# floe/backscrub

Measured on AMD Instinct MI355X. Metric: composited frames/sec at 640×480 (batch), 1/2/4/8 MI355X + mask IoU vs CPU ref, higher is better.
Workload: dtype f32 (network) / u8 (image kernels); 1 GPU; BASELINE configs[1]: batch=256 640x480 frames, segm_lite_v681.tflite; moving scene: ring of 4 batches, a new one every step; 1 step = prep+network+decode+mask+blend, inputs resident in HBM; streams_per_gpu=256, library=bsx 0.1 (HIP gfx950, f32 NHWC)

## Files before the change

backscrub_amd/csrc/bsx_api.hip:

```cpp
#include "debug_switches.hpp"
#include <hip/hip_runtime.h>

#include <algorithm>
#include <cmath>
#include <cstdarg>
#include <cstdio>
#include <cstdlib>
#include <cstring>
#include <map>
#include <memory>
#include <string>
#include <thread>
#include <vector>

#include "../../include/bsx.h"
#include "gen_mid.hpp"
#include "kernels.hpp"
#include "roctx_ranges.hpp"
#include "plan.hpp"
#include "refusal.hpp"
#include "rtc.hpp"
#include "specialised.hpp"
#include "tflite_model.hpp"

// ... 1721 lines not shown
    if (!load_tflite(model_path, &g, &err) || !build_plan(g, &p, &err)) { snprintf(msg, cap, "%s", err.c_str()); return BSX_EMODEL; }
    if (p.program.empty()) { snprintf(msg, cap, "interpreted (no program)"); return BSX_OK; }
    const SpecialisedBuild b = build_specialised(p, kernel_variant(p), arch ? arch : "gfx950");
    const std::string& e = b.mid.fallback;
    if (b.mid.code.empty()) { snprintf(msg, cap, "%s", e.c_str()); return e.compare(0, 19, "interpreted (hipRTC") == 0 ? BSX_EMODEL : BSX_OK; }
    std::string seg_msg;
    if (p.seg.on) {
      if (!b.seg.code.empty()) {
        long worst = 0;
        for (const char* k : {"bsx_seg_head", "bsx_seg_k2", "bsx_seg_k3", "bsx_seg_tail"}) worst = std::max(worst, code_object_scratch_bytes(b.seg.code, k));
        char sm[256];
        snprintf(sm, sizeof sm, "; segment kernels %s (%zu bytes of source, %zu bytes of code object, %ld B of scratch)", b.seg.cached ? "cached" : "compiled", b.seg.source.size(),
                 b.seg.code.size(), worst);
        seg_msg = sm;
      } else {
        seg_msg = "; segment kernels: " + b.seg.fallback;
        if (b.seg.fallback.find("hipRTC:") != std::string::npos) { snprintf(msg, cap, "%s", seg_msg.c_str()); return BSX_EMODEL; }
      }
    }
    snprintf(msg, cap, "%s (%zu bytes of source, %zu bytes of code object, %ld B of scratch%s, cache %s)%s", b.mid.cached ? "cached" : "compiled", b.mid.source.size(),
             b.mid.code.size(), b.scratch, b.opaque_tid ? ", lane indices re-derived per op" : "", rtc_cache_dir().c_str(), seg_msg.c_str());
    return BSX_OK;
  } catch (...) { snprintf(msg, cap, "exception while reading the model"); return BSX_EMODEL; }
}

const char* bsx_plan_describe(bsx_ctx* c) { return c ? c->plan_text.c_str() : ""; }

static const char* debug_tensor_unstored(const bsx_ctx* c, int t) {
  const Plan& p = c->plan;
  if (t == p.input) return nullptr;
  if (t == p.output) return c->last_net_logits ? nullptr : "the last network stage decoded inside its final kernel and wrote no logits";
  if (c->use_program) {
    if (p.seg.on && std::find(p.seg_stored.begin(), p.seg_stored.end(), t) != p.seg_stored.end()) return nullptr;
    for (size_t i = 0; i < p.program.size() && i < p.program_out_tensor.size(); i++) {
      if (p.program_out_tensor[i] != t) continue;
      if (p.program[i].out.space == kLocLds) return "the frame program keeps it in LDS";
      if (p.program[i].out.space != kLocGlobal) return "the frame program writes it to a buffer of its own";
      if (program_op_elided(c, (int)i)) return "the specialised middle kernel computes it chunk by chunk inside the depthwise that reads it";
      return nullptr;
    }
    return p.seg.on ? "it lives inside a segment kernel or a fused micro-op (LDS / registers only)" : "it lives inside a fused micro-op (LDS / registers only)";
  }
  const int NS = (int)p.steps.size();
  const int n = c->last_net_n > 0 ? c->last_net_n : c->n_streams;
  const bool ir_on = c->d_weights16 && c->f16_terms > 0;
  for (int j = 0; j < NS; j++) {
    const Step& st = p.steps[j];
    if (st.out != t) continue;
    if (p.steps[0].fuse_head0 && j < 2) return "the fused head kernel (stem + depthwise + 1x1) keeps it in LDS";
    if (st.fuse_dw >= 0 && ir_on) return "the fused expand + depthwise kernel keeps it in LDS";
    if (st.chain_first >= 0 && chain3_on(p, j, n, c->d_weights16, c->f16_terms)) return "the chained 1x1 kernel keeps it in registers";
    if (st.chain_mid >= 0 && j < st.chain_mid && chain3_on(p, st.chain_mid, n, c->d_weights16, c->f16_terms)) return "the chained 1x1 kernel keeps it in registers";
    return nullptr;
  }
  return "no step of this plan writes it";
}

static long debug_tensor_at(bsx_ctx* c, int t, int stream_idx, float* h_out, long cap) {
  if (!c) return BSX_EINVAL;
  if (t < 0 || t >= (int)c->plan.tensor_off.size() || t >= (int)c->plan.tensor_elems.size() || stream_idx < 0 || stream_idx >= c->n_streams || (h_out && cap < 0)) { c->last_error = "bsx_debug_tensor: tensor or stream index out of range"; return BSX_EINVAL; }
  if (c->plan.tensor_off[t] < 0) { c->last_error = "bsx_debug_tensor: tensor " + std::to_string(t) + " has no place in the arena (a constant, or fused away by the planner)"; return BSX_EINVAL; }
  if (const char* why = debug_tensor_unstored(c, t)) { c->last_error = "bsx_debug_tensor: tensor " + std::to_string(t) + " is never written to the arena on this path: " + why; return BSX_EINVAL; }
  DeviceGuard guard(c->device);
  const long n = c->plan.tensor_elems[t];
  if (!h_out) return n;
  const float* p = (t == c->plan.input || t == c->plan.output || !c->use_program) ? c->tensor_ptr(t) + (size_t)stream_idx * (size_t)n
// ... 20 lines not shown
```

backscrub_amd/csrc/gen_seg.cpp:

```cpp
#include "gen_seg.hpp"

#include <cstdarg>
#include <cstdio>

namespace bsx {
namespace {

const char kSegSource[] =
#include "seg_rtc_src.inc"
    ;

}

std::string seg_constants_text(const SegPlan& sp, const char* pre) {
  std::string out;
  auto P = [&](const char* fmt, ...) {
    char buf[1024];
    va_list ap;
    va_start(ap, fmt);
    vsnprintf(buf, sizeof buf, fmt, ap);
    va_end(ap);
    out += buf;
  };
  auto conv = [&](const char* n, const SegConvW& c) { P("  t.%s.w_off = %lldll; t.%s.b_off = %lldll; t.%s.Cin = %d; t.%s.Cout = %d; t.%s.cout_pad = %d; t.%s.act = %d;\n", n, c.w_off, n, c.b_off, n, c.Cin, n, c.Cout, n, c.cout_pad, n, c.act); };
  auto dw = [&](const char* n, const SegDwW& c) { P("  t.%s.w_off = %lldll; t.%s.b_off = %lldll; t.%s.C = %d; t.%s.act = %d;\n", n, c.w_off, n, c.b_off, n, c.C, n, c.act); };
  auto gate = [&](const char* n, const SegGate& g_) {
    P("  t.%s.n_parts = %d; t.%s.sum_parts = %d; t.%s.n_fc = %d; t.%s.timing_skip = %d;\n", n, g_.n_parts, n, g_.sum_parts, n, g_.n_fc, n, g_.timing_skip);
    for (int i = 0; i < 2; i++) {
      P("  t.%s.part[%d].off = %lldll; t.%s.part[%d].n = %d; t.%s.part[%d].C = %d; t.%s.part[%d].hw = (float)%.9g;\n", n, i, g_.part[i].off, n, i, g_.part[i].n, n, i, g_.part[i].C, n, i, (double)g_.part[i].hw);
      P("  t.%s.fc[%d].w_off = %lldll; t.%s.fc[%d].b_off = %lldll; t.%s.fc[%d].Cin = %d; t.%s.fc[%d].Cout = %d; t.%s.fc[%d].act = %d;\n", n, i, g_.fc[i].w_off, n, i, g_.fc[i].b_off, n, i, g_.fc[i].Cin, n, i,
              g_.fc[i].Cout, n, i, g_.fc[i].act);
    }
  };
  auto end = [&](int dbg_skip) { if (dbg_skip) P("  t.dbg_skip = %d;\n", dbg_skip); P("  return t; }();\n"); };
  const SegHead& H = sp.head; const SegK2& K2 = sp.k2; const SegK3& K3 = sp.k3; const SegTail& T = sp.tail;
  P("// segment descriptors of the loaded graph as constants (gen_seg.cpp: seg_constants_text)\nconstexpr SegHead %sHEAD = [] { SegHead t{};\n", pre);
  P("  t.H0 = %d; t.W0 = %d; t.H1 = %d; t.W1 = %d; t.H2 = %d; t.W2 = %d; t.stem_pt = %d; t.stem_pl = %d; t.dw_pt = %d; t.dw_pl = %d;\n", H.H0, H.W0, H.H1, H.W1, H.H2, H.W2, H.stem_pt, H.stem_pl, H.dw_pt, H.dw_pl);
  conv("stem", H.stem); conv("pw", H.pw); dw("dw", H.dw);
  P("  t.a_off = %lldll; t.b0_off = %lldll; t.part_a_off = %lldll; t.part_b0_off = %lldll; t.TR = %d; t.TC = %d; t.tiles_y = %d; t.tiles_x = %d; t.lds_floats = %d; t.rw = %d; t.m_ct = %uu;\n",
          H.a_off, H.b0_off, H.part_a_off, H.part_b0_off, H.TR, H.TC, H.tiles_y, H.tiles_x, H.lds_floats, H.rw, H.m_ct);
  end(H.dbg_skip);
  P("constexpr SegK2 %sK2 = [] { SegK2 t{};\n  t.H2 = %d; t.W2 = %d; t.H3 = %d; t.W3 = %d; t.dw_pt = %d; t.dw_pl = %d;\n", pre, K2.H2, K2.W2, K2.H3, K2.W3, K2.dw_pt, K2.dw_pl);
  gate("gate", K2.gate); conv("pw_a", K2.pw_a); conv("pw_b", K2.pw_b); dw("dw", K2.dw);
  P("  t.b0_off = %lldll; t.B_off = %lldll; t.c0_off = %lldll; t.part_B_off = %lldll; t.TR = %d; t.TC = %d; t.tiles_y = %d; t.tiles_x = %d; t.lds_floats = %d; t.rw = %d; t.m_ct = %uu;\n",
          K2.b0_off, K2.B_off, K2.c0_off, K2.part_B_off, K2.TR, K2.TC, K2.tiles_y, K2.tiles_x, K2.lds_floats, K2.rw, K2.m_ct);
  end(K2.dbg_skip);
  P("constexpr SegK3 %sK3 = [] { SegK3 t{};\n  t.H2 = %d; t.W2 = %d; t.HL = %d; t.WL = %d; t.half_pixel = %d; t.align_corners = %d;\n", pre, K3.H2, K3.W2, K3.HL, K3.WL, K3.half_pixel, K3.align_corners);
  conv("pw1", K3.pw1); conv("pw2", K3.pw2); dw("dw", K3.dw);
  P("  t.skip_off = %lldll; t.lo2_off = %lldll; t.g_off = %lldll; t.lo_off = %lldll; t.part_lo_off = %lldll; t.TR = %d; t.TC = %d; t.tiles_y = %d; t.tiles_x = %d; t.lds_floats = %d; t.lo_floats = %d; t.hs = (float)%.9g; t.ws = (float)%.9g;\n",
          K3.skip_off, K3.lo2_off, K3.g_off, K3.lo_off, K3.part_lo_off, K3.TR, K3.TC, K3.tiles_y, K3.tiles_x, K3.lds_floats, K3.lo_floats, (double)K3.hs, (double)K3.ws);
  end(K3.dbg_skip);
  P("constexpr SegTail %sTAIL = [] { SegTail t{};\n  t.H1 = %d; t.W1 = %d; t.HL = %d; t.WL = %d; t.H0 = %d; t.W0 = %d; t.half_pixel = %d; t.align_corners = %d;\n", pre, T.H1, T.W1, T.HL, T.WL, T.H0, T.W0, T.half_pixel, T.align_corners);
  gate("gate", T.gate); conv("pw", T.pw); dw("dw", T.dw);
  P("  t.tc_w_off = %lldll; t.tc_b_off = %lldll; t.Co = %d; t.act3 = %d; t.model_type = %d; t.skip_off = %lldll; t.lo_off = %lldll; t.pre_gate_off = %lldll; t.TR = %d; t.TC = %d; t.tiles_y = %d; t.tiles_x = %d; "
             "t.lds_floats = %d; t.lo_floats = %d; t.hs = (float)%.9g; t.ws = (float)%.9g;\n",
          T.tc_w_off, T.tc_b_off, T.Co, T.act3, T.model_type, T.skip_off, T.lo_off, T.pre_gate_off, T.TR, T.TC, T.tiles_y, T.tiles_x, T.lds_floats, T.lo_floats, (double)T.hs, (double)T.ws);
  end(T.dbg_skip);
  return out;
}

std::string generate_seg_source(const Plan& plan, bool h16, bool u8in, std::string* why) {
  auto fail = [&](const char* m) { if (why) *why = m; return std::string(); };
  if (!plan.seg.on) return fail("no segment kernels in this plan");
  const SegPlan& sp = plan.seg;
  const bool sig = sp.tail.act3 == kActSigmoid;
  if (!((sp.tail.Co == 2 && !sig) || sp.tail.Co == 1)) return fail("transpose-convolution output channels");
  std::string src = kSegSource;
  const std::string mark = "BSXS_SEG_CONSTANTS";
  const size_t at = src.find(mark);
  if (at == std::string::npos) return fail("embedded source has no constants marker");
  src.replace(at, mark.size(), seg_constants_text(sp, "kSeg"));
  char head[512];
  snprintf(head, sizeof head, "#define BSXS_SEG_RTC 1\n#define BSXS_SEG_HS %d\n#define BSXS_SEG_H16 %d\n#define BSXS_SEG_U8 %d\n#define BSXS_SEG_SIG %d\n#define BSXS_SEG_CO %d\n",
           sp.head.stem.act == kActHswish ? 1 : 0, h16 ? 1 : 0, u8in ? 1 : 0, sig ? 1 : 0, sp.tail.Co);
  return std::string(head) + src;
}

}
// ... 1 lines not shown
```

backscrub_amd/csrc/kernels_seg.hip:

```cpp
#ifndef __HIPCC_RTC__
#include <hip/hip_runtime.h>
#endif
#ifndef BSX_SEG_RTC
#include "debug_switches.hpp"

#include <algorithm>
#include <cstdlib>
#include <type_traits>

#include "kernels.hpp"
#include "mfma_tile.hpp"
#include "segments.hpp"
#endif

#if defined(BSX_SEG_RTC)
#define BSX_SEG_D(T, NAME) constexpr T d = kSeg##NAME; (void)d_rt
#elif defined(BSX_SEG_PROBE)
#define BSX_SEG_D(T, NAME) constexpr T d = kProbe##NAME; (void)d_rt
#else
#define BSX_SEG_D(T, NAME) const T& d = d_rt
#endif

namespace bsx {
#ifdef BSX_SEG_RTC
// ... 47 lines not shown
  c.hi = act == kActRelu6 ? 6.f : __builtin_huge_valf();
  return c;
}
__device__ __forceinline__ float4 clamp4(float4 v, Clamp c) {
  return make_float4(__builtin_amdgcn_fmed3f(v.x, c.lo, c.hi), __builtin_amdgcn_fmed3f(v.y, c.lo, c.hi), __builtin_amdgcn_fmed3f(v.z, c.lo, c.hi),
                     __builtin_amdgcn_fmed3f(v.w, c.lo, c.hi));
}
__device__ __forceinline__ float hswish1(float v) { return v * __builtin_amdgcn_fmed3f(v + 3.f, 0.f, 6.f) * 0.16666667163372040f; }
__device__ __forceinline__ float4 hswish4(float4 v) { return make_float4(hswish1(v.x), hswish1(v.y), hswish1(v.z), hswish1(v.w)); }
__device__ __forceinline__ float sigmoid1(float v) { return __builtin_amdgcn_rcpf(1.f + __builtin_amdgcn_exp2f(v * -1.44269504088896341f)); }
__device__ __forceinline__ float sg_act(float v, int act) {
  if (act == kActNone) return v;
  if (act == kActSigmoid) return sigmoid1(v);
  if (act == kActHswish) return hswish1(v);
  if (act == kActRelu) return fmaxf(v, 0.f);
  return __builtin_amdgcn_fmed3f(v, 0.f, 6.f);
}

__device__ __forceinline__ float4 acc_quad(const f4acc acc) { return make_float4(acc[0], acc[1], acc[2], acc[3]); }
__device__ __forceinline__ f4acc mma16(const float4 a, const float (&wr)[4]) {
  f4acc acc = {0.f, 0.f, 0.f, 0.f};
  acc = __builtin_amdgcn_mfma_f32_16x16x4f32(wr[0], a.x, acc, 0, 0, 0);
  acc = __builtin_amdgcn_mfma_f32_16x16x4f32(wr[1], a.y, acc, 0, 0, 0);
  acc = __builtin_amdgcn_mfma_f32_16x16x4f32(wr[2], a.z, acc, 0, 0, 0);
  acc = __builtin_amdgcn_mfma_f32_16x16x4f32(wr[3], a.w, acc, 0, 0, 0);
  return acc;
}
__device__ __forceinline__ void load_wtile(float (&wr)[4], const float* __restrict__ w, const SegConvW& c, int n0, int li, int g) {
#pragma unroll
  for (int r = 0; r < 4; r++) wr[r] = (w + c.w_off)[(unsigned)((4 * g + r) * c.cout_pad + n0 + li)];
}

constexpr int kGateStageFloats = kSegGateStageFloats;
__device__ __forceinline__ void seg_gate(const SegGate& gt, const float* __restrict__ fa, const float* __restrict__ w, float* scr, float* stage) {
  float* s_gate = scr + kScrGate;
  if (gt.timing_skip) { if (threadIdx.x < 16) s_gate[threadIdx.x] = 0.5f; __syncthreads(); return; }
  float* s_mean = scr + kScrGate + 16;
  float* s_hid = scr + kScrGate + 48;
  const int tid = threadIdx.x;
  const SegFc &f1 = gt.fc[0], &f2 = gt.fc[1];
  const int w1n = f1.Cin * f1.Cout, w2n = gt.n_fc == 2 ? f2.Cin * f2.Cout : 0;
  float* ps = stage;
  float* w1 = ps + 512;
  float* b1 = w1 + w1n;
  float* w2 = b1 + f1.Cout;
  float* b2 = w2 + w2n;
  {
    const int c = tid & 15, slice = tid >> 4;
    for (int k = 0; k < gt.n_parts; k++) {
      const float* src = fa + gt.part[k].off;
      float s = 0.f;
#pragma unroll 4
      for (int i = slice; i < gt.part[k].n; i += 16) s += src[(unsigned)(i * 16 + c)];
      ps[k * 256 + slice * 16 + c] = s;
    }
  }
  {
    const float* g1 = w + f1.w_off;
    const float* g2 = w + f2.w_off;
    for (int i = tid; i < w1n; i += kSegThreads) w1[i] = g1[(unsigned)i];
    for (int i = tid; i < w2n; i += kSegThreads) w2[i] = g2[(unsigned)i];
    if (tid < f1.Cout) b1[tid] = (w + f1.b_off)[(unsigned)tid];
    if (gt.n_fc == 2 && tid < f2.Cout) b2[tid] = (w + f2.b_off)[(unsigned)tid];
  }
  __syncthreads();
  const int Cm = gt.sum_parts ? 16 : 16 * gt.n_parts;
  if (tid < Cm) {
    float m = 0.f;
    for (int k = 0; k < gt.n_parts; k++) {
      if (!gt.sum_parts && (tid >> 4) != k) continue;
      float s = 0.f;
#pragma unroll
      for (int sl = 0; sl < 16; sl++) s += ps[k * 256 + sl * 16 + (tid & 15)];
      m += s / gt.part[k].hw;
    }
    s_mean[tid] = m;
  }
  __syncthreads();
  auto fc = [&](const SegFc& f, const float* x, const float* wl, const float* bl, float* y) {
    const int out = tid >> 3, ks = tid & 7, kper = f.Cin >> 3;
    float acc = 0.f;
    if (out < f.Cout)
      for (int j = 0; j < kper; j++) acc = fmaf(x[ks * kper + j], wl[out * f.Cin + ks * kper + j], acc);
    acc += dpp_quad(acc, 1);
    acc += dpp_quad(acc, 2);
    acc += __builtin_bit_cast(float, __builtin_amdgcn_update_dpp(0, __builtin_bit_cast(int, acc), 0x141, 0xf, 0xf, true));
    if (out < f.Cout && ks == 0) y[out] = sg_act(acc + bl[out], f.act);
  };
  fc(f1, s_mean, w1, b1, gt.n_fc == 1 ? s_gate : s_hid);
  __syncthreads();
  if (gt.n_fc == 2) {
    fc(f2, s_hid, w2, b2, s_gate);
    __syncthreads();
  }
}

template <int SHR>
// ... 197 lines not shown
    for (int s7 = 0; s7 < 7; s7++) {
      acc0 = __builtin_amdgcn_mfma_f32_16x16x4f32(ws[s7], av0[s7], acc0, 0, 0, 0);
      acc1 = __builtin_amdgcn_mfma_f32_16x16x4f32(ws[s7], av1[s7], acc1, 0, 0, 0);
    }
    stem_pw_epilogue(acc0, r0t);
    if (two) stem_pw_epilogue(acc1, r1t);
  }
  const int quad = lane & 3, px = lane >> 2;
  f4v wd[9];
#pragma unroll
  for (int k = 0; k < 9; k++) wd[k] = ldv(w + d.dw.w_off + k * 16 + 4 * quad);
  const f4v bias_d = ldv(w + d.dw.b_off + 4 * quad);
  const int cox[3] = {(2 * px) * 16 + 4 * quad, (2 * px + 1) * 16 + 4 * quad, (2 * px + 2) * 16 + 4 * quad};
  __syncthreads();

  float4 sumB = f4zero();
  for (int py = wave; py < d.TR && !(d.dbg_skip & 4); py += 4) {
    if (r0 + py >= d.H2) break;
    if (px < d.TC && c0 + px < d.W2) {
      const float4 v = as_stored<H16>(clamp4(tof4(dw3x3(x_f, AC * 16, 2 * py, cox, wd) + bias_d), cl_dw));
      stg4<H16>(b0_out, (unsigned)(((r0 + py) * d.W2 + c0 + px) * 16 + 4 * quad), v);
      sumB = f4add(sumB, v);
    }
  }
  float* s_red = in_t;
  wave_reduce16<0>(sumA, s_red, wave, lane);
  wave_reduce16<1>(sumB, s_red + 256, wave, lane);
  __syncthreads();
  store_partials(s_red, fa + d.part_a_off + (long)t_ * 16);
  store_partials(s_red + 256, fa + d.part_b0_off + (long)t_ * 16);
}

#ifdef BSX_SEG_RTC
extern "C" __global__ __launch_bounds__(kSegThreads) __attribute__((amdgpu_waves_per_eu(6, 6))) void bsx_seg_k2(
#else
template <bool H16>
__global__ __launch_bounds__(kSegThreads) __attribute__((amdgpu_waves_per_eu(6, 6))) void seg_k2_k(
#endif
    const SegK2 d_rt, float* __restrict__ arena, long per_frame, const float* __restrict__ w, int n_frames) {
  BSX_SEG_D(SegK2, K2);
  unsigned f_, t_;
  xcd_frame_tile((unsigned)(d.tiles_y * d.tiles_x), (unsigned)n_frames, &f_, &t_);
  const int f = (int)f_, ty = (int)t_ / d.tiles_x, tx = (int)t_ - ty * d.tiles_x;
  const int r0 = ty * d.TR, c0 = tx * d.TC;
  const int BR = 2 * d.TR + 1, BC = 2 * d.TC + 1, br0 = 2 * r0 - d.dw_pt, bc0 = 2 * c0 - d.dw_pl, RW = d.rw, ctiles = RW >> 4;
  float* fa = arena + (size_t)f * (size_t)per_frame;
  float* B_t = seg_smem + kScrFloats;
  float* x_t = B_t + BR * RW * 16;
  const float* b0_in = fa + d.b0_off;
  float* B_out = fa + d.B_off;
  float* c0_out = fa + d.c0_off;
  const int tid = threadIdx.x, lane = tid & 63, wave = wave_uniform(tid >> 6), li = lane & 15, g = lane >> 4, cq4 = 4 * g;
  const int ntile = BR * ctiles, xe = li;
  const int la = col_a(li, g), lb = col_b(li, g, RW >> 1);
  constexpr int kB0 = 6;
  float4 b0v[kB0];
#pragma unroll
  for (int j = 0; j < kB0; j++) {
    const int t = wave + 4 * j;
    b0v[j] = f4zero();
    if (t < ntile) {
      const RowTile rt = row_tile(t, ctiles, d.m_ct);
      const int gy = br0 + rt.row, gx = bc0 + 16 * rt.ct + li;
      if (gy >= 0 && gy < d.H2 && gx >= 0 && gx < d.W2) b0v[j] = ldg4<H16>(b0_in, (unsigned)((gy * d.W2 + gx) * 16 + 4 * g));
    }
  }
  seg_gate(d.gate, fa, w, seg_smem, B_t);
  const float4 sv = ld4(seg_smem + kScrGate + 4 * g);
  float wr[4];
  load_wtile(wr, w, d.pw_a, 0, li, g);
  const float4 bias_a = ld4(w + d.pw_a.b_off + cq4);
  const Clamp cl_a = clamp_of(d.pw_a.act), cl_b = clamp_of(d.pw_b.act), cl_dw = clamp_of(d.dw.act);

  float4 sumB = f4zero();
#pragma unroll
  for (int j = 0; j < kB0; j++) {
    const int t = wave + 4 * j;
    if (t >= ntile) break;
    const RowTile rt = row_tile(t, ctiles, d.m_ct);
    float4 a = b0v[j];
    a = make_float4(__fmul_rn(a.x, sv.x), __fmul_rn(a.y, sv.y), __fmul_rn(a.z, sv.z), __fmul_rn(a.w, sv.w));
    const f4acc acc = mma16(a, wr);
    float4 v = acc_quad(acc);
    const int x2 = 16 * rt.ct + xe, hy = br0 + rt.row, hx = bc0 + x2;
    if (x2 < BC) {
      v = as_stored<H16>(clamp4(f4add(v, bias_a), cl_a));
      st4(B_t + (rt.row * RW + 16 * rt.ct) * 16 + la, v);
      const bool row_owned = hy >= max(2 * r0, 0) && hy < min(2 * r0 + 2 * d.TR, d.H2);
      if (row_owned && hx >= 2 * c0 && hx < min(2 * c0 + 2 * d.TC, d.W2)) {
        stg4<H16>(B_out, (unsigned)((hy * d.W2 + hx) * 16 + cq4), v);
        sumB = f4add(sumB, v);
      }
    }
  }
  float* s_red = seg_smem + kScrRed;
  wave_reduce16<0>(sumB, s_red, wave, lane);
  __syncthreads();
  store_partials(s_red, fa + d.part_B_off + (long)t_ * 16);

  const int C = d.dw.C, ngrp = (C + 15) >> 4, quad = lane & 3, px = lane >> 2;
  const int cox[3] = {col_b(2 * px, quad, RW >> 1), col_b(2 * px + 1, quad, RW >> 1), col_b(2 * px + 2, quad, RW >> 1)};
  for (int grp = 0; grp < ngrp && !(d.dbg_skip & 2); grp++) {
    load_wtile(wr, w, d.pw_b, 16 * grp, li, g);
    const float4 bias_b = ld4(w + d.pw_b.b_off + 16 * grp + cq4);
    for (int t = wave; t < ntile; t += 4) {
      const RowTile rt = row_tile(t, ctiles, d.m_ct);
      const f4acc acc = mma16(ld4(B_t + (rt.row * RW + 16 * rt.ct) * 16 + la), wr);
      float4 v = acc_quad(acc);
      const int x2 = 16 * rt.ct + xe, hy = br0 + rt.row, hx = bc0 + x2;
      if (x2 < BC) {
        const bool inside = hy >= 0 && hy < d.H2 && hx >= 0 && hx < d.W2;
        v = inside ? clamp4(f4add(v, bias_b), cl_b) : f4zero();
        st4(x_t + (rt.row * RW + 8 * rt.ct) * 16 + lb, v);
      }
    }
    const int ch = 16 * grp + 4 * quad;
    f4v wd[9];
    f4v bias_d = {0.f, 0.f, 0.f, 0.f};
    if (ch < C) {
#pragma unroll
      for (int k = 0; k < 9; k++) wd[k] = ldv(w + d.dw.w_off + (unsigned)(k * C + ch));
      bias_d = ldv(w + d.dw.b_off + ch);
    }
    __syncthreads();
    if (ch < C && px < d.TC && c0 + px < d.W3)
      for (int py = wave; py < d.TR && r0 + py < d.H3; py += 4) {
        const float4 v = clamp4(tof4(dw3x3(x_t, RW * 16, 2 * py, cox, wd) + bias_d), cl_dw);
        stg4<H16>(c0_out, (unsigned)(((r0 + py) * d.W3 + c0 + px) * C + ch), v);
      }
    __syncthreads();
  }
}

constexpr int kGatedRows = 5;
constexpr int kLoStride = kSegLoStride;
struct GatedPre { float4 s[kGatedRows]; int ly0, lx0, LC; };
template <bool H16>
__device__ __forceinline__ GatedPre gated_prefetch(const float* __restrict__ skip, const float* __restrict__ lo, int H, int W, int HL, int WL, bool half_pixel,
                                                   float hs, float wsc, int r0, int c0, int ZH, int ZC, float* l_t) {
  const int tid = threadIdx.x, lane = tid & 63, wave = wave_uniform(tid >> 6), li = lane & 15, g = lane >> 4;
  GatedPre pre;
  const int ix = c0 - 1 + li;
  const bool col_in = li < ZC && ix >= 0 && ix < W;
#pragma unroll
  for (int j = 0; j < kGatedRows; j++) {
    const int zy = wave + 4 * j, iy = r0 - 1 + zy;
    pre.s[j] = f4zero();
    if (zy < ZH && iy >= 0 && iy < H && col_in) pre.s[j] = ldg4<H16>(skip, (unsigned)((iy * W + ix) * 16 + 4 * g));
  }
  int ly0, ly1, lx0, lx1, t0, t1;
  float fr;
  up_axis(max(r0 - 1, 0), hs, half_pixel, HL, &ly0, &t1, &fr);
  up_axis(min(r0 - 2 + ZH, H - 1), hs, half_pixel, HL, &t0, &ly1, &fr);
  up_axis(max(c0 - 1, 0), wsc, half_pixel, WL, &lx0, &t1, &fr);
  up_axis(min(c0 - 2 + ZC, W - 1), wsc, half_pixel, WL, &t0, &lx1, &fr);
  const int LR = ly1 - ly0 + 1, LC = lx1 - lx0 + 1;
  pre.ly0 = ly0; pre.lx0 = lx0; pre.LC = LC;
  float4 v[3];
#pragma unroll
  for (int j = 0; j < 3; j++) {
    const int ly = wave + 4 * j;
    v[j] = f4zero();
// ... 265 lines not shown
```

backscrub_amd/csrc/plan.cpp:

```cpp
#include "debug_switches.hpp"
#include "plan.hpp"
#include "gen_seg.hpp"
#include "gen_mid.hpp"

#include <algorithm>
#include <cmath>
#include <cstdio>
#include <cstdlib>
#include <cstring>
#include <map>

namespace bsx {
namespace {

void conv_geometry(int in, int k, int s, int d, bool same, int* out, int* pad) {
  int eff = (k - 1) * d + 1;
  *out = same ? (in + s - 1) / s : (in + s - eff) / s;
  int total = (*out - 1) * s + eff - in;
  *pad = total > 0 ? total / 2 : 0;
}

uint16_t f32_to_f16_rn(float f) {
  uint32_t x; memcpy(&x, &f, 4);
  const uint32_t sign = (x >> 16) & 0x8000u;
// ... 564 lines not shown
  if (uses_of(B) != 3 || uses_of(up2) != 2 || uses_of(kp1.out) != 2 || uses_of(kd.out) != 1 || uses_of(kf2.out) != 1 || uses_of(lo) != 1 || uses_of(lo2) != 1) return seg_fail(21);
  if (!resize_weights_uniform(kr.H, kr.OH, kr.align_corners, kr.half_pixel) || !resize_weights_uniform(kr.W, kr.OW, kr.align_corners, kr.half_pixel)) return seg_fail(22);
  if (uses_of(c0) != 1) return seg_fail(23);
  auto clampish = [](int a) { return a == kActNone || a == kActRelu || a == kActRelu6; };
  if (!(clampish(stem.act) || stem.act == kActHswish) || !(ttc.act == kActNone || ttc.act == kActSigmoid) || (ttc.act == kActSigmoid && ttc.Cout != 1)) return seg_fail(34);
  for (const Step* q : {&hpw, &hdw, &pwa, &pwb, &kdw, &kp1, &kd, &kp2, &tpw, &tdw}) if (!clampish(q->act)) return seg_fail(35);

  size_t top = plan->arena_floats_per_stream;
  auto reserve = [&](size_t floats) { size_t at = top; top += (floats + 63) / 64 * 64; return (long long)at; };
  auto synth = [&](const char* name, int n, int C) {
    TensorInfo t; t.dims[0] = 1; t.dims[1] = n; t.dims[2] = 1; t.dims[3] = C; t.shape = {1, n, 1, C}; t.name = name;
    g.tensors.push_back(t);
    plan->tensor_off.push_back(-1);
    return (int)g.tensors.size() - 1;
  };
  SegPlan sp;
  int tgt[8] = {4, 14, 4, 7, 16, 14, 18, 14};
  if (const char* e = BSX_DBG_ENV("BSX_SEG_TILES")) sscanf(e, "%d,%d,%d,%d,%d,%d,%d,%d", &tgt[0], &tgt[1], &tgt[2], &tgt[3], &tgt[4], &tgt[5], &tgt[6], &tgt[7]);
  auto split = [&](int extent, int target, int* tile, int* n) { *n = tiles_for(extent, std::max(1, target)); *tile = (extent + *n - 1) / *n; };

  SegHead& h = sp.head;
  h.H0 = stem.H; h.W0 = stem.W; h.H1 = stem.OH; h.W1 = stem.OW; h.H2 = hdw.OH; h.W2 = hdw.OW;
  h.stem_pt = stem.pad_t; h.stem_pl = stem.pad_l; h.dw_pt = hdw.pad_t; h.dw_pl = hdw.pad_l;
  h.stem = conv_w(stem); h.pw = conv_w(hpw); h.dw = dw_w(hdw);
  split(h.H2, tgt[0], &h.TR, &h.tiles_y); split(h.W2, tgt[1], &h.TC, &h.tiles_x);
  h.lds_floats = seg_head_lds_floats(h);
  h.rw = seg_row_width(2 * h.TC + 1); h.m_ct = (65536u + (unsigned)(h.rw / 16) - 1) / (unsigned)(h.rw / 16);
  if (h.TR > 4 || h.TC > 15 || (4 * h.TC + 3) * 3 > 192) return seg_fail(30);
  SegK2& k2 = sp.k2;
  k2.H2 = hdw.OH; k2.W2 = hdw.OW; k2.H3 = kdw.OH; k2.W3 = kdw.OW; k2.dw_pt = kdw.pad_t; k2.dw_pl = kdw.pad_l;
  k2.pw_a = conv_w(pwa); k2.pw_b = conv_w(pwb); k2.dw = dw_w(kdw);
  split(k2.H3, tgt[2], &k2.TR, &k2.tiles_y); split(k2.W3, tgt[3], &k2.TC, &k2.tiles_x);
  k2.lds_floats = seg_k2_lds_floats(k2);
  k2.rw = seg_row_width(2 * k2.TC + 1); k2.m_ct = (65536u + (unsigned)(k2.rw / 16) - 1) / (unsigned)(k2.rw / 16);
  if (k2.TC > 15 || ((2 * k2.TR + 1) * (k2.rw / 16) + 3) / 4 > 6) return seg_fail(31);
  SegK3& k3 = sp.k3;
  k3.H2 = kp1.OH; k3.W2 = kp1.OW; k3.HL = kr.H; k3.WL = kr.W; k3.half_pixel = kr.half_pixel; k3.align_corners = kr.align_corners;
  k3.pw1 = conv_w(kp1); k3.pw2 = conv_w(kp2); k3.dw = dw_w(kd);
  split(k3.H2, tgt[4], &k3.TR, &k3.tiles_y); split(k3.W2, tgt[5], &k3.TC, &k3.tiles_x);
  k3.hs = seg_up_scale(k3.HL, k3.H2, k3.align_corners != 0); k3.ws = seg_up_scale(k3.WL, k3.W2, k3.align_corners != 0);
  if (!BSX_DBG_ENV("BSX_SEG_LO_WORST")) k3.lo_floats = seg_lo_window_floats(k3.H2, k3.W2, k3.HL, k3.WL, k3.half_pixel != 0, k3.align_corners != 0, k3.TR, k3.TC, k3.tiles_y, k3.tiles_x);
  k3.lds_floats = seg_k3_lds_floats(k3);
  if (k3.TC > 14 || k3.TR > 18) return seg_fail(32);
  SegTail& tl = sp.tail;
  tl.H1 = tpw.OH; tl.W1 = tpw.OW; tl.HL = tr.H; tl.WL = tr.W; tl.H0 = ttc.OH; tl.W0 = ttc.OW; tl.half_pixel = tr.half_pixel; tl.align_corners = tr.align_corners;
  tl.pw = conv_w(tpw); tl.dw = dw_w(tdw); tl.tc_w_off = (long long)ttc.w_off; tl.tc_b_off = (long long)ttc.b_off; tl.Co = ttc.Cout; tl.act3 = ttc.act;
  split(tl.H1, tgt[6], &tl.TR, &tl.tiles_y); split(tl.W1, tgt[7], &tl.TC, &tl.tiles_x);
  tl.hs = seg_up_scale(tl.HL, tl.H1, tl.align_corners != 0); tl.ws = seg_up_scale(tl.WL, tl.W1, tl.align_corners != 0);
  if (!BSX_DBG_ENV("BSX_SEG_LO_WORST")) tl.lo_floats = seg_lo_window_floats(tl.H1, tl.W1, tl.HL, tl.WL, tl.half_pixel != 0, tl.align_corners != 0, tl.TR, tl.TC, tl.tiles_y, tl.tiles_x);
  tl.lds_floats = seg_tail_lds_floats(tl);
  if (tl.TC > 14 || tl.TR > 18) return seg_fail(33);
  const int lds_cap = 160 * 256;
  if (h.lds_floats > lds_cap || k2.lds_floats > lds_cap || k3.lds_floats > lds_cap || tl.lds_floats > lds_cap) return seg_fail(24);
  if (ttc.OH != 2 * tpw.OH || ttc.OW != 2 * tpw.OW || h.H2 != k3.H2 || h.W2 != k3.W2) return seg_fail(25);
  if (h.tiles_y * h.tiles_x > 1024 || k2.tiles_y * k2.tiles_x > 1024 || k3.tiles_y * k3.tiles_x > 1024) return seg_fail(26);

  const int pA = synth("partials(A)", h.tiles_y * h.tiles_x, 16), pb0 = synth("partials(b0)", h.tiles_y * h.tiles_x, 16);
  const int pB = synth("partials(B)", k2.tiles_y * k2.tiles_x, 16), plo = synth("partials(lo)", k3.tiles_y * k3.tiles_x, 16);
  const int pgt = BSX_DBG_ENV("BSX_SEG_NO_GATE_KERNEL") ? -1 : synth("gate(tail)", 1, 16);
  if (pgt >= 0) plan->tensor_off[pgt] = reserve(16);
  for (int t : {A, b0, B, c0, lo2, lo, kf2.out, pA, pb0, pB, plo}) plan->tensor_off[t] = reserve(g.tensors[t].elems());
  for (int t : {hpw.out, g1.out, f1a.out, f1b.out, pwb.out, up2, kg.out, kf1.out, kp1.out, kd.out, up, tg.out, tf1.out, tf2.out, tpw.out, tdw.out})
    if (t != g.output) plan->tensor_off[t] = -1;
  plan->arena_floats_per_stream = top;
  plan->seg_stored = {A, b0, B, c0, lo};

  h.a_off = plan->tensor_off[A]; h.b0_off = plan->tensor_off[b0]; h.part_a_off = plan->tensor_off[pA]; h.part_b0_off = plan->tensor_off[pb0];
  k2.b0_off = plan->tensor_off[b0]; k2.B_off = plan->tensor_off[B]; k2.c0_off = plan->tensor_off[c0]; k2.part_B_off = plan->tensor_off[pB];
  k2.gate.n_parts = 1; k2.gate.n_fc = 2; k2.gate.sum_parts = 0;
  k2.gate.part[0].off = plan->tensor_off[pb0]; k2.gate.part[0].n = h.tiles_y * h.tiles_x; k2.gate.part[0].C = 16; k2.gate.part[0].hw = (float)(h.H2 * h.W2);
  k2.gate.fc[0] = fc_w(f1a); k2.gate.fc[1] = fc_w(f1b);
  k3.skip_off = plan->tensor_off[B]; k3.lo2_off = plan->tensor_off[lo2]; k3.g_off = plan->tensor_off[kf2.out]; k3.lo_off = plan->tensor_off[lo];
  k3.part_lo_off = plan->tensor_off[plo];
  tl.skip_off = plan->tensor_off[A]; tl.lo_off = plan->tensor_off[lo];
  tl.gate.n_parts = 2; tl.gate.n_fc = 2; tl.gate.sum_parts = tg.gap_sum ? 1 : 0;
  tl.gate.part[0].off = plan->tensor_off[pA]; tl.gate.part[0].n = h.tiles_y * h.tiles_x; tl.gate.part[0].C = 16; tl.gate.part[0].hw = (float)(h.H1 * h.W1);
  tl.gate.part[1].off = plan->tensor_off[plo]; tl.gate.part[1].n = k3.tiles_y * k3.tiles_x; tl.gate.part[1].C = 16; tl.gate.part[1].hw = (float)(k3.H2 * k3.W2);
  tl.gate.fc[0] = fc_w(tf1); tl.gate.fc[1] = fc_w(tf2);
  if (BSX_DBG_ENV("BSX_SEG_GATE_SKIP")) k2.gate.timing_skip = tl.gate.timing_skip = 1;
  if (const char* e = BSX_DBG_ENV("BSX_SEG_SKIP")) sscanf(e, "%d,%d,%d,%d", &h.dbg_skip, &k2.dbg_skip, &k3.dbg_skip, &tl.dbg_skip);
  tl.pre_gate_off = pgt >= 0 ? plan->tensor_off[pgt] : -1;
  if (tl.gate.fc[0].Cin != (tl.gate.sum_parts ? 16 : 32) || k2.gate.fc[0].Cin != 16) return seg_fail(27);

  std::vector<Step> mid(S.begin() + 9, S.begin() + (NS - 14));
  Step gate = kg;
  gate.concat_in = {B, lo2};
  gate.in0 = B;
  gate.label += "*";
  mid.push_back(gate); mid.push_back(kf1); mid.push_back(kf2);
  std::map<int, int> part_n, part_hw;
  part_n[B] = k2.tiles_y * k2.tiles_x; part_hw[B] = k2.H2 * k2.W2;
  const long B_real = plan->tensor_off[B];
  plan->tensor_off[B] = plan->tensor_off[pB];
  build_frame_program(g, plan, mid, {c0, B, lo2, kf2.out}, part_n, part_hw);
  plan->tensor_off[B] = B_real;
  if (plan->program.empty()) return seg_fail(28);
  sp.on = true;
  plan->seg = sp;
#ifdef BSX_DEBUG_SWITCHES
  if (const char* path = BSX_DBG_ENV("BSX_SEG_DUMP")) {
    if (FILE* f = fopen(path, "w")) { fputs(seg_constants_text(sp, "kProbe").c_str(), f); fclose(f); }
  }
#endif
  char line[256];
  plan->seg_text.clear();
  auto add = [&](const char* name, int TR, int TC, int ty, int tx, int lds, std::initializer_list<int> stores) {
    snprintf(line, sizeof line, "segment %-5s tile %dx%d, %dx%d tiles per frame, LDS %.1f KiB, stores", name, TR, TC, ty, tx, lds / 256.0);
    plan->seg_text += line;
    for (int t : stores) plan->seg_text += " t" + std::to_string(t);
    plan->seg_text += stores.size() ? "\n" : " the network output\n";
  };
  add("head", h.TR, h.TC, h.tiles_y, h.tiles_x, h.lds_floats, {A, b0}); add("k2", k2.TR, k2.TC, k2.tiles_y, k2.tiles_x, k2.lds_floats, {B, c0});
  add("k3", k3.TR, k3.TC, k3.tiles_y, k3.tiles_x, k3.lds_floats, {lo}); add("tail", tl.TR, tl.TC, tl.tiles_y, tl.tiles_x, tl.lds_floats, {});
  return true;
}


MidGeometry mid_geometry_default() {
  static const MidGeometry geo = [] {
    MidGeometry m{kFrameThreads, kLdsTotalFloats};
    if (const char* e = BSX_DBG_ENV("BSX_MID_LANES")) { const int v = atoi(e); if (v == 512 || v == 1024) m.lanes = v; }
    if (const char* e = BSX_DBG_ENV("BSX_MID_LDS_KB")) { const int v = atoi(e); if (v >= 64 && v <= 160) m.lds_floats = v * 256; }
    return m;
  }();
  return geo;
}

bool build_plan(const Graph& g_in, Plan* plan, std::string* err, bool reuse_arena, bool segments) {
  auto fail = [&](const std::string& m) { if (err) *err = m; return false; };
  { const MidGeometry geo = mid_geometry_default(); plan->mid_lanes = geo.lanes; plan->lds_total_floats = geo.lds_floats; }
  Graph g = g_in;
  int NT = (int)g.tensors.size();
  const int NN = (int)g.nodes.size();

  std::vector<std::vector<int>> users(NT);
  for (int i = 0; i < NN; i++) for (int t : g.nodes[i].inputs) if (t >= 0 && !g.tensors[t].is_const) users[t].push_back(i);
  auto single_user = [&](int t) -> int { return (t != g.output && users[t].size() == 1) ? users[t][0] : -1; };

  std::vector<char> fused(NN, 0);
  std::vector<Step> steps;
  std::vector<float>& W = plan->weights;
  W.clear();
  auto align_w = [&]() { while (W.size() % 4) W.push_back(0.f); };

  for (int i = 0; i < NN; i++) {
    if (fused[i]) continue;
// ... 513 lines not shown
```

backscrub_amd/csrc/plan.hpp:

```cpp
#pragma once
#include "debug_switches.hpp"
#include <cstdio>
#include <cstdlib>
#include <cstddef>
#include <string>
#include <vector>

#include "frame_program.hpp"
#include "segments.hpp"
#include "tflite_model.hpp"

namespace bsx {

enum class StepKind : int { Conv = 0, PwConv, DwConv, Gap, Eltwise, Resize, Concat, TConv };
enum EltOp : int { kEltAdd = 0, kEltMul = 1, kEltUnary = 2, kEltMulAdd = 3 };

struct Step {
  StepKind kind = StepKind::Conv;
  std::string label;
  int in0 = -1, in1 = -1, in2 = -1;
  int out = -1;
  int residual = -1;
  int in_scale = -1;
  int out_bias = -1;
// ... 67 lines not shown
    if (head0_lds_floats(W0, W1, bh) * 4 <= 80 * 1024) return bh;
  for (int bh = 8; bh >= 2; bh--)
    if (head0_lds_floats(W0, W1, bh) * 4 <= 156 * 1024) return bh;
  return 0;
}

struct Plan {
  std::vector<Step> steps;
  std::vector<float> weights;
  std::vector<uint16_t> weights16;
  std::vector<long> tensor_off;
  std::vector<long> tensor_elems;
  size_t arena_floats_per_stream = 0;
  int input = -1, output = -1;
  double macs_per_frame = 0;
  std::vector<MicroOp> program;
  std::vector<std::string> program_labels;
  std::vector<int> program_out_tensor;
  int mid_lanes = kFrameThreads;
  int lds_total_floats = kLdsTotalFloats;
  int lds_zero_off() const { return lds_total_floats - kLdsZeroFloats; }
  int program_lds_floats = 0;
  int program_scratch_floats = 0;
  int program_lds_tensors = 0, program_global_tensors = 0;
  std::vector<long> program_ext_offs;
  struct LdsBlock { int off, len, from, until; std::string what; };
  std::vector<LdsBlock> program_blocks;
  std::string program_check;
  SegPlan seg;
  unsigned program_policy = 0;
  long program_arena_bytes = 0;
  std::string seg_text;
  std::vector<int> seg_stored;
  std::string describe() const;
};

struct MidGeometry { int lanes, lds_floats; };
MidGeometry mid_geometry_default();

std::string verify_program_lds(const Plan& plan);

bool build_plan(const Graph& g, Plan* plan, std::string* err, bool reuse_arena = true, bool segments = true);

}
```

backscrub_amd/csrc/segments.hpp:

```cpp
#pragma once
#ifndef BSX_SEG_RTC
#include <algorithm>
#include <cmath>
#include <cstdint>
#endif

namespace bsx {

struct SegConvW { long long w_off = 0, b_off = 0; int Cin = 0, Cout = 0, cout_pad = 0, act = 0; };
struct SegDwW { long long w_off = 0, b_off = 0; int C = 0, act = 0; };
struct SegFc { long long w_off = 0, b_off = 0; int Cin = 0, Cout = 0, act = 0; };
struct SegPart { long long off = 0; int n = 0, C = 0; float hw = 1.f; };
struct SegGate {
  int n_parts = 0, sum_parts = 0, n_fc = 0;
  int timing_skip = 0;
  SegPart part[2];
  SegFc fc[2];
};

constexpr int kSegThreads = 256;
constexpr int kSegMaxC = 16;

struct SegHead {
  int H0 = 0, W0 = 0, H1 = 0, W1 = 0, H2 = 0, W2 = 0;
  int stem_pt = 0, stem_pl = 0, dw_pt = 0, dw_pl = 0;
  SegConvW stem, pw;
  SegDwW dw;
  long long a_off = 0, b0_off = 0, part_a_off = 0, part_b0_off = 0;
  int TR = 0, TC = 0, tiles_y = 0, tiles_x = 0;
  int lds_floats = 0;
  int dbg_skip = 0;
  int rw = 0;
  unsigned m_ct = 0;
};

struct SegK2 {
  int H2 = 0, W2 = 0, H3 = 0, W3 = 0;
  int dw_pt = 0, dw_pl = 0;
  SegGate gate;
  SegConvW pw_a, pw_b;
  SegDwW dw;
  long long b0_off = 0, B_off = 0, c0_off = 0, part_B_off = 0;
  int TR = 0, TC = 0, tiles_y = 0, tiles_x = 0;
  int lds_floats = 0;
  int dbg_skip = 0;
  int rw = 0;
  unsigned m_ct = 0;
};

struct SegK3 {
  int H2 = 0, W2 = 0, HL = 0, WL = 0;
  int half_pixel = 0, align_corners = 0;
  SegConvW pw1, pw2;
  SegDwW dw;
  long long skip_off = 0, lo2_off = 0, g_off = 0, lo_off = 0, part_lo_off = 0;
  int TR = 0, TC = 0, tiles_y = 0, tiles_x = 0;
  int lds_floats = 0;
  int lo_floats = 0;
  float hs = 0.f, ws = 0.f;
  int dbg_skip = 0;
};

struct SegTail {
  int H1 = 0, W1 = 0, HL = 0, WL = 0, H0 = 0, W0 = 0;
  int half_pixel = 0, align_corners = 0;
  SegGate gate;
  SegConvW pw;
  SegDwW dw;
  long long tc_w_off = 0, tc_b_off = 0;
  int Co = 0, act3 = 0, model_type = 0;
  long long skip_off = 0, lo_off = 0;
  long long pre_gate_off = -1;
  int TR = 0, TC = 0, tiles_y = 0, tiles_x = 0;
  int lds_floats = 0;
  int lo_floats = 0;
  float hs = 0.f, ws = 0.f;
  int dbg_skip = 0;
};

constexpr int kSegLoStride = 16;
constexpr int kSegLoTileFloats = 12 * 16 * kSegLoStride;
constexpr int kSegScratchFloats = 640;
constexpr int kSegGateStageFloats = 512 + 2 * (32 * 32 + 32);
#ifndef BSX_SEG_RTC
inline int seg_row_width(int cols) { return (cols + 15) / 16 * 16; }
inline int seg_head_lds_floats(const SegHead& d) {
  const int AR = 2 * d.TR + 1, AC = 2 * d.TC + 1, IR = 2 * AR + 1, IC = 2 * AC + 1;
  const int win = (IR * IC * 3 + 3) & ~3;
  return (win > 512 ? win : 512) + AR * AC * 16;
}
inline int seg_k2_lds_floats(const SegK2& d) { const int v = 2 * (2 * d.TR + 1) * seg_row_width(2 * d.TC + 1) * 16; return kSegScratchFloats + (v > kSegGateStageFloats ? v : kSegGateStageFloats); }
inline void seg_up_axis(int o, float scale, bool half_pixel, int in_size, int* lo, int* hi) {
  const float v = half_pixel ? ((float)o + 0.5f) * scale + -0.5f : (float)o * scale;
  const float fl = std::floor(v);
  *lo = std::max((int)fl, 0);
  *hi = std::min((int)std::ceil(v), in_size - 1);
}
inline float seg_up_scale(int in, int out, bool align) { return (align && out > 1) ? (float)(in - 1) / (float)(out - 1) : (float)in / (float)out; }
inline int seg_lo_window_floats(int H, int W, int HL, int WL, bool half_pixel, bool align, int TR, int TC, int tiles_y, int tiles_x) {
  const float hs = seg_up_scale(HL, H, align), ws = seg_up_scale(WL, W, align);
  int lr = 1, lc = 1, a, b, c, e;
  for (int ty = 0; ty < tiles_y; ty++) {
    const int r0 = ty * TR;
    seg_up_axis(std::max(r0 - 1, 0), hs, half_pixel, HL, &a, &b);
    seg_up_axis(std::min(r0 + TR, H - 1), hs, half_pixel, HL, &c, &e);
    lr = std::max(lr, e - a + 1);
  }
  for (int tx = 0; tx < tiles_x; tx++) {
    const int c0 = tx * TC;
    seg_up_axis(std::max(c0 - 1, 0), ws, half_pixel, WL, &a, &b);
    seg_up_axis(std::min(c0 + TC, W - 1), ws, half_pixel, WL, &c, &e);
    lc = std::max(lc, e - a + 1);
  }
  const int need = (lr + 1) * (lc + 1) * kSegLoStride;
  return need < kSegLoTileFloats ? need : kSegLoTileFloats;
}
inline int seg_k3_lds_floats(const SegK3& d) { return kSegScratchFloats + (d.TR + 2) * 256 + (d.lo_floats > 0 ? d.lo_floats : kSegLoTileFloats); }
inline int seg_tail_lds_floats(const SegTail& d) { const int v = (d.TR + 2) * 256; return kSegScratchFloats + (v > kSegGateStageFloats ? v : kSegGateStageFloats) + (d.lo_floats > 0 ? d.lo_floats : kSegLoTileFloats); }
#endif

struct SegPlan {
  bool on = false;
  SegHead head;
  SegK2 k2;
// ... 6 lines not shown
```

Baseline: 716,700 frames/s.

## Stage k2 pointwise and depthwise weights in LDS with double-buffered prefetch

The k2 segment kernel now copies the pw_b weight tile and bias per channel group into a double-buffered LDS area, and optionally the depthwise weights and bias too. The next group's weights are prefetched into registers during the current group's work. The first group's stores are hidden inside the gate's existing barrier through a publish callback. The planner adds staging only when the extra LDS does not lower the number of workgroups per CU, and also records partial-sum tensors for debug output. The aim is to take repeated global weight loads off the inner loop. The cost is extra LDS, register pressure and more complex code.

After: 726,400 frames/s (median of 6 runs). +1.4%, better.

```diff
diff --git a/backscrub_amd/csrc/bsx_api.hip b/backscrub_amd/csrc/bsx_api.hip
--- a/backscrub_amd/csrc/bsx_api.hip
+++ b/backscrub_amd/csrc/bsx_api.hip
@@ -1777,6 +1777,7 @@
   if (t == p.output) return c->last_net_logits ? nullptr : "the last network stage decoded inside its final kernel and wrote no logits";
   if (c->use_program) {
     if (p.seg.on && std::find(p.seg_stored.begin(), p.seg_stored.end(), t) != p.seg_stored.end()) return nullptr;
+    if (p.seg.on && std::find(p.seg_partials.begin(), p.seg_partials.end(), t) != p.seg_partials.end()) return nullptr;
     for (size_t i = 0; i < p.program.size() && i < p.program_out_tensor.size(); i++) {
       if (p.program_out_tensor[i] != t) continue;
       if (p.program[i].out.space == kLocLds) return "the frame program keeps it in LDS";
diff --git a/backscrub_amd/csrc/gen_seg.cpp b/backscrub_amd/csrc/gen_seg.cpp
--- a/backscrub_amd/csrc/gen_seg.cpp
+++ b/backscrub_amd/csrc/gen_seg.cpp
@@ -44,6 +44,8 @@
   gate("gate", K2.gate); conv("pw_a", K2.pw_a); conv("pw_b", K2.pw_b); dw("dw", K2.dw);
   P("  t.b0_off = %lldll; t.B_off = %lldll; t.c0_off = %lldll; t.part_B_off = %lldll; t.TR = %d; t.TC = %d; t.tiles_y = %d; t.tiles_x = %d; t.lds_floats = %d; t.rw = %d; t.m_ct = %uu;\n",
           K2.b0_off, K2.B_off, K2.c0_off, K2.part_B_off, K2.TR, K2.TC, K2.tiles_y, K2.tiles_x, K2.lds_floats, K2.rw, K2.m_ct);
+  P("  t.wst.form = %d; t.wst.off = %d; t.wst.floats = %d; t.wst.stride = %d; t.wst.buf_floats = %d; t.wst.bias_off = %d; t.wst.dw_off = %d; t.wst.dwb_off = %d;\n",
+          K2.wst.form, K2.wst.off, K2.wst.floats, K2.wst.stride, K2.wst.buf_floats, K2.wst.bias_off, K2.wst.dw_off, K2.wst.dwb_off);
   end(K2.dbg_skip);
   P("constexpr SegK3 %sK3 = [] { SegK3 t{};\n  t.H2 = %d; t.W2 = %d; t.HL = %d; t.WL = %d; t.half_pixel = %d; t.align_corners = %d;\n", pre, K3.H2, K3.W2, K3.HL, K3.WL, K3.half_pixel, K3.align_corners);
   conv("pw1", K3.pw1); conv("pw2", K3.pw2); dw("dw", K3.dw);
diff --git a/backscrub_amd/csrc/kernels_seg.hip b/backscrub_amd/csrc/kernels_seg.hip
--- a/backscrub_amd/csrc/kernels_seg.hip
+++ b/backscrub_amd/csrc/kernels_seg.hip
@@ -103,9 +103,11 @@
 }
 
 constexpr int kGateStageFloats = kSegGateStageFloats;
-__device__ __forceinline__ void seg_gate(const SegGate& gt, const float* __restrict__ fa, const float* __restrict__ w, float* scr, float* stage) {
+struct NoPublish { __device__ __forceinline__ void operator()() const {} };
+template <class Publish = NoPublish>
+__device__ __forceinline__ void seg_gate(const SegGate& gt, const float* __restrict__ fa, const float* __restrict__ w, float* scr, float* stage, Publish publish = Publish()) {
   float* s_gate = scr + kScrGate;
-  if (gt.timing_skip) { if (threadIdx.x < 16) s_gate[threadIdx.x] = 0.5f; __syncthreads(); return; }
+  if (gt.timing_skip) { if (threadIdx.x < 16) s_gate[threadIdx.x] = 0.5f; publish(); __syncthreads(); return; }
   float* s_mean = scr + kScrGate + 16;
   float* s_hid = scr + kScrGate + 48;
   const int tid = threadIdx.x;
@@ -134,6 +136,7 @@
     if (tid < f1.Cout) b1[tid] = (w + f1.b_off)[(unsigned)tid];
     if (gt.n_fc == 2 && tid < f2.Cout) b2[tid] = (w + f2.b_off)[(unsigned)tid];
   }
+  publish();
   __syncthreads();
   const int Cm = gt.sum_parts ? 16 : 16 * gt.n_parts;
   if (tid < Cm) {
@@ -397,10 +400,10 @@
 }
 
 #ifdef BSX_SEG_RTC
-extern "C" __global__ __launch_bounds__(kSegThreads) __attribute__((amdgpu_waves_per_eu(6, 6))) void bsx_seg_k2(
+extern "C" __global__ __launch_bounds__(kSegThreads) __attribute__((amdgpu_waves_per_eu(kSegK2Waves, kSegK2Waves))) void bsx_seg_k2(
 #else
 template <bool H16>
-__global__ __launch_bounds__(kSegThreads) __attribute__((amdgpu_waves_per_eu(6, 6))) void seg_k2_k(
+__global__ __launch_bounds__(kSegThreads) __attribute__((amdgpu_waves_per_eu(kSegK2Waves, kSegK2Waves))) void seg_k2_k(
 #endif
     const SegK2 d_rt, float* __restrict__ arena, long per_frame, const float* __restrict__ w, int n_frames) {
   BSX_SEG_D(SegK2, K2);
@@ -412,6 +415,10 @@
   float* fa = arena + (size_t)f * (size_t)per_frame;
   float* B_t = seg_smem + kScrFloats;
   float* x_t = B_t + BR * RW * 16;
+#ifdef BSX_SEG_RTC
+  static_assert(d.wst.form == 0 || (d.wst.off >= kScrFloats + 2 * BR * RW * 16 && d.wst.off >= kScrFloats + kGateStageFloats && d.wst.off + d.wst.floats == d.lds_floats),
+                "k2: staged weights outside the planned LDS");
+#endif
   const float* b0_in = fa + d.b0_off;
   float* B_out = fa + d.B_off;
   float* c0_out = fa + d.c0_off;
@@ -430,11 +437,48 @@
       if (gy >= 0 && gy < d.H2 && gx >= 0 && gx < d.W2) b0v[j] = ldg4<H16>(b0_in, (unsigned)((gy * d.W2 + gx) * 16 + 4 * g));
     }
   }
-  seg_gate(d.gate, fa, w, seg_smem, B_t);
+#ifdef BSX_SEG_RTC
+  constexpr SegStage st = d.wst;
+#else
+  const SegStage st{};
+#endif
+  float* sw = seg_smem + st.off;
+  auto pwb_fetch = [&](int grp) {
+    float4 v = f4zero();
+    if (tid < 64) v = ld4(w + d.pw_b.w_off + (unsigned)((tid & 15) * d.pw_b.cout_pad + 16 * grp + 4 * (tid >> 4)));
+    else if (tid < 68) v = ld4(w + d.pw_b.b_off + 16 * grp + 4 * (tid - 64));
+    return v;
+  };
+  auto pwb_store = [&](int buf, float4 v) {
+    float* dst = sw + buf * st.buf_floats;
+    if (tid < 64) st4(dst + (tid & 15) * st.stride + 4 * (tid >> 4), v);
+    else if (tid < 68) st4(dst + st.bias_off + 4 * (tid - 64), v);
+  };
+  float wr[4];
+  float4 bias_a, sf[3];
+  if (st.form >= 1) {
+    load_wtile(wr, w, d.pw_a, 0, li, g);
+    bias_a = ld4(w + d.pw_a.b_off + cq4);
+    sf[0] = pwb_fetch(0);
+    if (st.form >= 2) {
+      if (4 * tid < 9 * d.dw.C) sf[1] = ld4(w + d.dw.w_off + 4 * tid);
+      if (4 * tid < d.dw.C) sf[2] = ld4(w + d.dw.b_off + 4 * tid);
+    }
+  }
+  seg_gate(d.gate, fa, w, seg_smem, B_t, [&] {
+    if (st.form >= 1) {
+      pwb_store(0, sf[0]);
+      if (st.form >= 2) {
+        if (4 * tid < 9 * d.dw.C) st4(sw + st.dw_off + 4 * tid, sf[1]);
+        if (4 * tid < d.dw.C) st4(sw + st.dwb_off + 4 * tid, sf[2]);
+      }
+    }
+  });
   const float4 sv = ld4(seg_smem + kScrGate + 4 * g);
-  float wr[4];
-  load_wtile(wr, w, d.pw_a, 0, li, g);
-  const float4 bias_a = ld4(w + d.pw_a.b_off + cq4);
+  if (st.form == 0) {
+    load_wtile(wr, w, d.pw_a, 0, li, g);
+    bias_a = ld4(w + d.pw_a.b_off + cq4);
+  }
   const Clamp cl_a = clamp_of(d.pw_a.act), cl_b = clamp_of(d.pw_b.act), cl_dw = clamp_of(d.dw.act);
 
   float4 sumB = f4zero();
@@ -466,8 +510,17 @@
   const int C = d.dw.C, ngrp = (C + 15) >> 4, quad = lane & 3, px = lane >> 2;
   const int cox[3] = {col_b(2 * px, quad, RW >> 1), col_b(2 * px + 1, quad, RW >> 1), col_b(2 * px + 2, quad, RW >> 1)};
   for (int grp = 0; grp < ngrp && !(d.dbg_skip & 2); grp++) {
-    load_wtile(wr, w, d.pw_b, 16 * grp, li, g);
-    const float4 bias_b = ld4(w + d.pw_b.b_off + 16 * grp + cq4);
+    float4 bias_b, nxt;
+    if (st.form >= 1) {
+      const float* tb = sw + (grp & 1) * st.buf_floats;
+#pragma unroll
+      for (int r = 0; r < 4; r++) wr[r] = tb[(4 * g + r) * st.stride + li];
+      bias_b = ld4(tb + st.bias_off + cq4);
+      if (grp + 1 < ngrp) nxt = pwb_fetch(grp + 1);
+    } else {
+      load_wtile(wr, w, d.pw_b, 16 * grp, li, g);
+      bias_b = ld4(w + d.pw_b.b_off + 16 * grp + cq4);
+    }
     for (int t = wave; t < ntile; t += 4) {
       const RowTile rt = row_tile(t, ctiles, d.m_ct);
       const f4acc acc = mma16(ld4(B_t + (rt.row * RW + 16 * rt.ct) * 16 + la), wr);
@@ -482,10 +535,14 @@
     const int ch = 16 * grp + 4 * quad;
     f4v wd[9];
     f4v bias_d = {0.f, 0.f, 0.f, 0.f};
-    if (ch < C) {
+    if (ch < C && st.form < 2) {
 #pragma unroll
       for (int k = 0; k < 9; k++) wd[k] = ldv(w + d.dw.w_off + (unsigned)(k * C + ch));
       bias_d = ldv(w + d.dw.b_off + ch);
+    } else if (ch < C) {
+#pragma unroll
+      for (int k = 0; k < 9; k++) wd[k] = ldv(sw + st.dw_off + k * C + ch);
+      bias_d = ldv(sw + st.dwb_off + ch);
     }
     __syncthreads();
     if (ch < C && px < d.TC && c0 + px < d.W3)
@@ -493,6 +550,7 @@
         const float4 v = clamp4(tof4(dw3x3(x_t, RW * 16, 2 * py, cox, wd) + bias_d), cl_dw);
         stg4<H16>(c0_out, (unsigned)(((r0 + py) * d.W3 + c0 + px) * C + ch), v);
       }
+    if (st.form >= 1 && grp + 1 < ngrp) pwb_store((grp + 1) & 1, nxt);
     __syncthreads();
   }
 }
diff --git a/backscrub_amd/csrc/plan.cpp b/backscrub_amd/csrc/plan.cpp
--- a/backscrub_amd/csrc/plan.cpp
+++ b/backscrub_amd/csrc/plan.cpp
@@ -620,6 +620,8 @@
   k2.pw_a = conv_w(pwa); k2.pw_b = conv_w(pwb); k2.dw = dw_w(kdw);
   split(k2.H3, tgt[2], &k2.TR, &k2.tiles_y); split(k2.W3, tgt[3], &k2.TC, &k2.tiles_x);
   k2.lds_floats = seg_k2_lds_floats(k2);
+  k2.wst = seg_k2_stage(k2, k2.lds_floats, dbg_env_int(BSX_DBG_ENV("BSX_K2_LDS_CAP"), 160 * 1024), BSX_DBG_ENV("BSX_K2_GLOBAL_W") ? 0 : 2);
+  k2.lds_floats += k2.wst.floats;
   k2.rw = seg_row_width(2 * k2.TC + 1); k2.m_ct = (65536u + (unsigned)(k2.rw / 16) - 1) / (unsigned)(k2.rw / 16);
   if (k2.TC > 15 || ((2 * k2.TR + 1) * (k2.rw / 16) + 3) / 4 > 6) return seg_fail(31);
   SegK3& k3 = sp.k3;
@@ -651,6 +653,7 @@
   for (int t : {hpw.out, g1.out, f1a.out, f1b.out, pwb.out, up2, kg.out, kf1.out, kp1.out, kd.out, up, tg.out, tf1.out, tf2.out, tpw.out, tdw.out})
     if (t != g.output) plan->tensor_off[t] = -1;
   plan->arena_floats_per_stream = top;
+  plan->seg_partials = {pA, pb0, pB, plo};
   plan->seg_stored = {A, b0, B, c0, lo};
 
   h.a_off = plan->tensor_off[A]; h.b0_off = plan->tensor_off[b0]; h.part_a_off = plan->tensor_off[pA]; h.part_b0_off = plan->tensor_off[pb0];
@@ -690,16 +693,21 @@
     if (FILE* f = fopen(path, "w")) { fputs(seg_constants_text(sp, "kProbe").c_str(), f); fclose(f); }
   }
 #endif
-  char line[256];
+  char line[256], k2_note[64] = "";
   plan->seg_text.clear();
   auto add = [&](const char* name, int TR, int TC, int ty, int tx, int lds, std::initializer_list<int> stores) {
-    snprintf(line, sizeof line, "segment %-5s tile %dx%d, %dx%d tiles per frame, LDS %.1f KiB, stores", name, TR, TC, ty, tx, lds / 256.0);
+    snprintf(line, sizeof line, "segment %-5s tile %dx%d, %dx%d tiles per frame, LDS %.1f KiB%s, stores", name, TR, TC, ty, tx, lds / 256.0, k2_note);
     plan->seg_text += line;
     for (int t : stores) plan->seg_text += " t" + std::to_string(t);
     plan->seg_text += stores.size() ? "\n" : " the network output\n";
   };
-  add("head", h.TR, h.TC, h.tiles_y, h.tiles_x, h.lds_floats, {A, b0}); add("k2", k2.TR, k2.TC, k2.tiles_y, k2.tiles_x, k2.lds_floats, {B, c0});
+  add("head", h.TR, h.TC, h.tiles_y, h.tiles_x, h.lds_floats, {A, b0});
+  snprintf(k2_note, sizeof k2_note, " (weights staged: form %d, %d B)", k2.wst.form, k2.wst.floats * 4);
+  add("k2", k2.TR, k2.TC, k2.tiles_y, k2.tiles_x, k2.lds_floats, {B, c0});
+  k2_note[0] = 0;
   add("k3", k3.TR, k3.TC, k3.tiles_y, k3.tiles_x, k3.lds_floats, {lo}); add("tail", tl.TR, tl.TC, tl.tiles_y, tl.tiles_x, tl.lds_floats, {});
+  snprintf(line, sizeof line, "segment partial sums ([tiles][16] f32): A t%d, b0 t%d, B t%d, lo t%d\n", pA, pb0, pB, plo);
+  plan->seg_text += line;
   return true;
 }
 
diff --git a/backscrub_amd/csrc/plan.hpp b/backscrub_amd/csrc/plan.hpp
--- a/backscrub_amd/csrc/plan.hpp
+++ b/backscrub_amd/csrc/plan.hpp
@@ -123,6 +123,7 @@
   long program_arena_bytes = 0;
   std::string seg_text;
   std::vector<int> seg_stored;
+  std::vector<int> seg_partials;
   std::string describe() const;
 };
 
diff --git a/backscrub_amd/csrc/segments.hpp b/backscrub_amd/csrc/segments.hpp
--- a/backscrub_amd/csrc/segments.hpp
+++ b/backscrub_amd/csrc/segments.hpp
@@ -19,6 +19,7 @@
 };
 
 constexpr int kSegThreads = 256;
+constexpr int kSegK2Waves = 6;
 constexpr int kSegMaxC = 16;
 
 struct SegHead {
@@ -34,6 +35,8 @@
   unsigned m_ct = 0;
 };
 
+struct SegStage { int form = 0, off = 0, floats = 0, stride = 0, buf_floats = 0, bias_off = 0, dw_off = 0, dwb_off = 0; };
+
 struct SegK2 {
   int H2 = 0, W2 = 0, H3 = 0, W3 = 0;
   int dw_pt = 0, dw_pl = 0;
@@ -46,6 +49,7 @@
   int dbg_skip = 0;
   int rw = 0;
   unsigned m_ct = 0;
+  SegStage wst;
 };
 
 struct SegK3 {
@@ -90,6 +94,27 @@
   return (win > 512 ? win : 512) + AR * AC * 16;
 }
 inline int seg_k2_lds_floats(const SegK2& d) { const int v = 2 * (2 * d.TR + 1) * seg_row_width(2 * d.TC + 1) * 16; return kSegScratchFloats + (v > kSegGateStageFloats ? v : kSegGateStageFloats); }
+constexpr int kSegStageStride = 20;
+inline int seg_k2_wgs_per_cu(int lds_floats, int lds_cap_bytes) { const int by_lds = lds_cap_bytes / (lds_floats * 4); return by_lds < kSegK2Waves ? by_lds : kSegK2Waves; }
+inline SegStage seg_k2_stage(const SegK2& d, int base_floats, int lds_cap_bytes, int max_form) {
+  SegStage best;
+  const int wgs0 = seg_k2_wgs_per_cu(base_floats, lds_cap_bytes);
+  const int ncol = (d.dw.C + 15) / 16 * 16, C = d.dw.C;
+  const bool ok1 = ncol <= d.pw_b.cout_pad && d.pw_b.Cin == 16 && d.pw_b.w_off % 4 == 0 && d.pw_b.b_off % 4 == 0 && d.pw_b.cout_pad % 4 == 0;
+  const bool ok2 = ok1 && C % 4 == 0 && 9 * C / 4 <= kSegThreads && d.dw.w_off % 4 == 0 && d.dw.b_off % 4 == 0;
+  for (int form = 1; form <= 2 && form <= max_form; form++) {
+    if (!(form == 1 ? ok1 : ok2)) break;
+    SegStage s;
+    s.form = form; s.off = base_floats; s.stride = kSegStageStride;
+    s.bias_off = 16 * s.stride;
+    s.buf_floats = s.bias_off + 16;
+    s.floats = 2 * s.buf_floats;
+    if (form == 2) { s.dw_off = s.floats; s.dwb_off = s.dw_off + 9 * C; s.floats = s.dwb_off + C; }
+    if (wgs0 < 1 || seg_k2_wgs_per_cu(base_floats + s.floats, lds_cap_bytes) != wgs0) break;
+    best = s;
+  }
+  return best;
+}
 inline void seg_up_axis(int o, float scale, bool half_pixel, int in_size, int* lo, int* hi) {
   const float v = half_pixel ? ((float)o + 0.5f) * scale + -0.5f : (float)o * scale;
   const float fl = std::floor(v);
```
